# baurst/liso

Hardware: AMD Instinct MI355X
Metric: LISO train-step frames/sec (120k-pt clouds) (higher is better)
Workload: dtype bf16 (detector, BASELINE configs[2]) + f32 via bf16x3 MFMA (SLIM); north_star's 1e-3 on logits / flow is met by `parity_leg` (f32 via bf16x3 MFMA everywhere) and `fp32_exact_leg`, not by the bf16 detector

## Files before the change

liso_amd/csrc/conv_mfma.hip:

```cpp
#include <hip/hip_runtime.h>
#include <stdint.h>
#include <stdlib.h>

#include "../../include/liso_conv.h"
#include "../../include/liso_iou3d.h"
#include "conv_plan.h"
#include "dev_common.h"
#include "elem16.h"
#include "pack_chunk.h"
#include "per_device.h"

namespace {

using liso_dev::check_launch;

typedef __bf16 bf8 __attribute__((ext_vector_type(8)));
typedef float f16v __attribute__((ext_vector_type(16)));

__device__ __forceinline__ int xcd_remap(int bid, int total) {
    const int q = total >> 3, r = total & 7;
    const int xcd = bid & 7, idx = bid >> 3;
    return (xcd < r ? xcd * (q + 1) : r * (q + 1) + (xcd - r) * q) + idx;
}

using liso_pack::pack_bf16;
using liso_pack::round_bf16;
__device__ __forceinline__ float bf16_lo(unsigned w) { return __uint_as_float(w << 16); }
__device__ __forceinline__ float bf16_hi(unsigned w) { return __uint_as_float(w & 0xffff0000u); }

__device__ __forceinline__ bf8 as_bf8(const uint4& v) { return __builtin_bit_cast(bf8, v); }

template <typename E, int MI, int NJ, bool OUT_F32, bool WAVE_STATS = false>
__device__ __forceinline__ void conv_epilogue(const liso_conv_desc& d, const FwdArgs& a, f16v (&acc)[MI][NJ], int cls, int b, int tx, int ty,
                                              int wave, int r, int h, bool active, int n0, int stats_row, int tid_all,
                                              unsigned char* smem) {
    constexpr int BNT = 32 * NJ;
    constexpr int TH = 4 * MI;
    const int tid = tid_all & (kThreads - 1);
    const int grp = active ? 0 : 1;
    const bool want_stats = a.stats != nullptr;
    float s1[NJ], s2[NJ];
    const int ooy = d.class_ooy[cls], oox = d.class_oox[cls];
    const int col_stride = d.osx * d.y_pix_stride;
    unsigned colmask = 0;
#pragma unroll
    for (int e = 0; e < 16; e++) {
        const int vx = tx * 32 + (e & 3) + 8 * (e >> 2) + 4 * h;
        if (vx < d.wv && vx * d.osx + oox < d.wo) colmask |= 1u << e;
    }
    const int col0 = (tx * 32 + 4 * h) * d.osx + oox;
#pragma unroll
    for (int j = 0; j < NJ; j++) {
        s1[j] = 0.0f;
        s2[j] = 0.0f;
    }
#pragma unroll
    for (int i = 0; i < MI; i++) {
        const int vy = ty * TH + wave * MI + i;
        const int oy = vy * d.osy + ooy;
        const unsigned rowmask = (grp == 0 && vy < d.hv && oy < d.ho) ? colmask : 0u;
        if constexpr (WAVE_STATS) {
#pragma unroll
            for (int j = 0; j < NJ; j++) {
                s1[j] = 0.0f;
                s2[j] = 0.0f;
            }
        }
        const long row_base = (((long)b * d.ho + oy) * d.wo + col0) * d.y_pix_stride + d.y_ch_off;
#pragma unroll
        for (int j = 0; j < NJ; j++) {
            const int n = n0 + j * 32 + r;
            const bool n_ok = n < d.co;
            const float bias_v = (a.bias && n_ok) ? a.bias[n] : 0.0f;
            const float shift_v = (a.stats_shift && n_ok) ? a.stats_shift[n] : 0.0f;
            float v[16];
#pragma unroll
            for (int e = 0; e < 16; e++) {
                float val = acc[i][j][e] + bias_v;
                if (d.out_relu) val = fmaxf(val, 0.0f);
                if constexpr (!OUT_F32) val = E::round(val);
                v[e] = val;
                if constexpr (!WAVE_STATS) {
                    if (want_stats && ((rowmask >> e) & 1u)) {
                        const float dd = val - shift_v;
                        s1[j] += dd;
                        s2[j] = fmaf(dd, dd, s2[j]);
                    }
                }
            }
            if constexpr (WAVE_STATS) {
                if (want_stats) {
                    float q1[16], q2[16];
#pragma unroll
                    for (int e = 0; e < 16; e++) {
                        const float dd = ((rowmask >> e) & 1u) ? v[e] - shift_v : 0.0f;
                        q1[e] = dd;
                        q2[e] = dd * dd;
                    }
#pragma unroll
                    for (int w = 8; w >= 1; w >>= 1)
#pragma unroll
                        for (int e = 0; e < w; e++) {
                            q1[e] += q1[e + w];
                            q2[e] += q2[e + w];
                        }
                    s1[j] = q1[0];
                    s2[j] = q2[0];
                }
            }
            if constexpr (OUT_F32) {
                float* yg = (float*)a.y + row_base + n;
#pragma unroll
                for (int e = 0; e < 16; e++)
                    if (((rowmask >> e) & 1u) && n_ok) yg[((e & 3) + 8 * (e >> 2)) * col_stride] = v[e];
            } else {
                unsigned short* yg = (unsigned short*)a.y + row_base;
                const bool odd = r & 1;
                const int n_even = n & ~1;
                if ((d.y_pix_stride | d.y_ch_off) & 1) {
#pragma unroll
                    for (int e = 0; e < 16; e++)
                        if (((rowmask >> e) & 1u) && n_ok)
                            yg[((e & 3) + 8 * (e >> 2)) * col_stride + n] = (unsigned short)(E::pack(v[e], 0.0f) & 0xffffu);
                } else {
#pragma unroll
                    for (int e = 0; e < 16; e += 2) {
                        const float send = odd ? v[e] : v[e + 1];
                        const float recv = __int_as_float(__builtin_amdgcn_mov_dpp(__float_as_int(send), 0xB1, 0xF, 0xF, true));
                        const float c_lo = odd ? recv : v[e];
                        const float c_hi = odd ? v[e + 1] : recv;
                        const int ee = odd ? e + 1 : e;
                        const int koff = odd ? ((e + 1) & 3) + 8 * ((e + 1) >> 2) : (e & 3) + 8 * (e >> 2);
                        if ((rowmask >> ee) & 1u) {
                            unsigned short* dst = yg + koff * col_stride + n_even;
                            if (n_even + 1 < d.co)
                                *reinterpret_cast<unsigned*>(dst) = E::pack(c_lo, c_hi);
                            else if (n_even < d.co)
                                *dst = (unsigned short)(E::pack(c_lo, 0.0f) & 0xffffu);
                        }
                    }
                }
            }
        }
        if constexpr (WAVE_STATS) {
            if (want_stats) {
                float* red = reinterpret_cast<float*>(smem);
#pragma unroll
                for (int j = 0; j < NJ; j++) {
                    const float t1 = s1[j] + __shfl_xor(s1[j], 32);
                    const float t2 = s2[j] + __shfl_xor(s2[j], 32);
                    if (h == 0) {
                        red[((wave * MI + i) * BNT + j * 32 + r) * 2 + 0] = t1;
                        red[((wave * MI + i) * BNT + j * 32 + r) * 2 + 1] = t2;
                    }
                }
            }
        }
    }
    if constexpr (WAVE_STATS) {
    } else if (want_stats) {
        float* red = reinterpret_cast<float*>(smem);
#pragma unroll
        for (int j = 0; j < NJ; j++) {
            const float t1 = s1[j] + __shfl_xor(s1[j], 32);
            const float t2 = s2[j] + __shfl_xor(s2[j], 32);
            if (h == 0 && grp == 0) {
                red[(wave * BNT + j * 32 + r) * 2 + 0] = t1;
                red[(wave * BNT + j * 32 + r) * 2 + 1] = t2;
            }
        }
        __syncthreads();
        if (tid_all < BNT && n0 + tid < a.co_pad) {
            float q1 = 0.0f, q2 = 0.0f;
#pragma unroll
            for (int w = 0; w < 4; w++) {
                q1 += red[(w * BNT + tid) * 2 + 0];
                q2 += red[(w * BNT + tid) * 2 + 1];
            }
            a.stats[((long)stats_row * 2 + 0) * a.co_pad + n0 + tid] = q1;
            a.stats[((long)stats_row * 2 + 1) * a.co_pad + n0 + tid] = q2;
        }
    }
}
// ... 766 lines not shown
                }
            }
        };
        auto mul = [&](const Frag& F) {
#pragma unroll
            for (int kk = 0; kk < KS; kk++)
#pragma unroll
                for (int i = 0; i < MI; i++)
#pragma unroll
                    for (int j = 0; j < NJ; j++) {
                        if constexpr (X3) {
                            acc[i][j] = __builtin_amdgcn_mfma_f32_32x32x16_bf16(as_bf8(F.al[kk][i]), as_bf8(F.bh[kk][j]), acc[i][j], 0, 0, 0);
                            acc[i][j] = __builtin_amdgcn_mfma_f32_32x32x16_bf16(as_bf8(F.ah[kk][i]), as_bf8(F.bl[kk][j]), acc[i][j], 0, 0, 0);
                        }
                        acc[i][j] = E::mfma(F.ah[kk][i], F.bh[kk][j], acc[i][j]);
                    }
        };
#ifdef LISO_ROLES_STAMPS
        unsigned long long st_mul = 0, st_bar = 0, st_epi = 0, st_t;
        const unsigned long long st_k0 = __builtin_amdgcn_s_memtime();
#endif
        barrier();
#ifdef LISO_ROLES_STAMPS
        const unsigned long long st_k1 = __builtin_amdgcn_s_memtime();
#endif
        int k = 0;
        for (int j = 0; j < my_tiles; j++) {
#pragma unroll
            for (int i = 0; i < MI; i++)
#pragma unroll
                for (int jj = 0; jj < NJ; jj++)
#pragma unroll
                    for (int e = 0; e < 16; e++) acc[i][jj][e] = 0.0f;
            __builtin_amdgcn_s_setprio(2);
            for (int sl = 0; sl < nslab; sl++, k++) {
                const unsigned char* buf = base + (k & 1) * BUF;
                Frag F0, F1;
                STAMP_BEGIN
                read(buf, 0, F0);
#pragma unroll
                for (int tp = 0; tp < NTAPS; tp += 2) {
                    if (tp + 1 < NTAPS) read(buf, tp + 1, F1);
                    __builtin_amdgcn_sched_barrier(0);
                    mul(F0);
                    __builtin_amdgcn_sched_barrier(0);
                    if (tp + 1 < NTAPS) {
                        if (tp + 2 < NTAPS) read(buf, tp + 2, F0);
                        __builtin_amdgcn_sched_barrier(0);
                        mul(F1);
                        __builtin_amdgcn_sched_barrier(0);
                    }
                }
                STAMP_END(st_mul)
                barrier();
                STAMP_END(st_bar)
#ifndef LISO_ROLES_STAMPS
                if (sl == 0 && j > 0 && a.stats) {
                    const Tile P = tile_of(j - 1);
                    roles_flush_stats<MI, NJ>(a, P.b, P.ty, P.tx, P.n0, tid_all, smem);
                }
#endif
            }
            __builtin_amdgcn_s_setprio(0);
            const Tile T = tile_of(j);
#ifdef LISO_ROLES_STAMPS
            FwdArgs a2 = a;
            a2.stats = nullptr;
            conv_epilogue<E, MI, NJ, OUT_F32, true>(d, a2, acc, 0, T.b, T.tx, T.ty, wave, r, h, true, T.n0, T.row, tid_all, smem);
            STAMP_END(st_epi)
#else
            if (a.wide_out)
                roles_epilogue<E, MI, NJ, OUT_F32>(d, a, acc, T.b, T.tx, T.ty, wave, lane, T.n0, smem, base + 2 * BUF + wave * 2048);
            else
                conv_epilogue<E, MI, NJ, OUT_F32, true>(d, a, acc, 0, T.b, T.tx, T.ty, wave, r, h, true, T.n0, T.row, tid_all, smem);
#endif
        }
#ifndef LISO_ROLES_STAMPS
        if (a.stats) {
            barrier();
            const Tile P = tile_of(my_tiles - 1);
            roles_flush_stats<MI, NJ>(a, P.b, P.ty, P.tx, P.n0, tid_all, smem);
        }
#else
        if (a.stats) barrier();
#endif
#ifdef LISO_ROLES_STAMPS
        if (a.stats && tid_all == 0) {
            unsigned long long* o = reinterpret_cast<unsigned long long*>(a.stats) + (size_t)blockIdx.x * 16;
            o[0] = st_k1 - st_k0; o[1] = st_mul; o[2] = st_bar; o[3] = __builtin_amdgcn_s_memtime() - st_k0; o[4] = st_epi;
        }
#endif
    }
}

template <int MODE, int MI, int NJ, bool OUT_F32, bool PRO>
__global__ __launch_bounds__(kThreads, 2) void conv_1x1_kernel(const liso_conv_desc d, const FwdArgs a) {
    using E = typename liso_e16::Elem<MODE>::T;
    constexpr bool X3 = MODE == LISO_CONV_F32X3;
    constexpr int BNT = 32 * NJ;
    constexpr int TH = 4 * MI;
    constexpr int ES = X3 ? 4 : 2;
    __shared__ __attribute__((aligned(16))) unsigned char smem[4 * 96 * 2 * 4];
    __shared__ int s_dy[LISO_CONV_MAX_TAPS], s_dx[LISO_CONV_MAX_TAPS], s_w[LISO_CONV_MAX_TAPS];
    const int tid_all = threadIdx.x, wave = tid_all >> 6, lane = tid_all & 63, r = lane & 31, h = lane >> 5;
    if (tid_all < d.n_taps) {
        s_dy[tid_all] = d.tap_dy[tid_all];
        s_dx[tid_all] = d.tap_dx[tid_all];
        s_w[tid_all] = d.tap_w[tid_all];
    }
    int t = xcd_remap(blockIdx.x, a.total);
    const int nt = t % a.n_nt;
    t /= a.n_nt;
    const int tx = t % a.tiles_x;
    t /= a.tiles_x;
    const int ty = t % a.tiles_y;
    t /= a.tiles_y;
    const int b = t % d.batch;
    const int cls = t / d.batch;
    const int stats_row = ((cls * d.batch + b) * a.tiles_y + ty) * a.tiles_x + tx;
    const int n0 = nt * BNT;
    const int tap0 = d.n_classes > 1 ? cls : 0, tap1 = d.n_classes > 1 ? cls + 1 : d.n_taps;
    const unsigned char* xb = (const unsigned char*)a.x + (long)b * d.hi * d.wi * d.x_pix_stride * ES;
    int by[MI];
    bool okv[MI];
    const int bx = (tx * 32 + r) * d.isx;
#pragma unroll
    for (int i = 0; i < MI; i++) {
        const int vy = ty * TH + wave * MI + i;
        okv[i] = vy < d.hv && tx * 32 + r < d.wv;
        by[i] = vy * d.isy;
    }
    const unsigned short* wg = (const unsigned short*)a.w;
    const int kgroups = a.ci_pad >> 3;
    const long plane_elems = (long)d.w_taps * kgroups * a.co_pad * 8;
    int wn[NJ];
    bool okn[NJ];
#pragma unroll
    for (int j = 0; j < NJ; j++) {
        const int n = n0 + j * 32 + r;
        okn[j] = n < a.co_pad;
        wn[j] = (okn[j] ? n : 0) * 8;
    }
    const int aff = b * d.in_affine_batch_stride;
    __syncthreads();
    struct Frag {
        uint4 x[MI][X3 ? 2 : 1];
        float4 sc[2], sh[2];
        uint4 bh[NJ], bl[X3 ? NJ : 1];
        unsigned ok;
    };
    const int K = a.ci_pad;
    const int n_steps = (tap1 - tap0) * (K >> 4);
    int cur_tap = tap0, cur_k = 0;
    auto load = [&](Frag& F) {
        const int c = cur_k + 8 * h;
        const bool v0 = c < d.ci, v1 = c + 4 < d.ci;
        const int c_lo = v0 ? c : 0, c_hi = v1 ? c + 4 : 0;
        const int dy = s_dy[cur_tap], dx = s_dx[cur_tap];
        const int ix = bx + dx;
        unsigned ok = (v0 ? 256u : 0u) | (v1 ? 512u : 0u);
#pragma unroll
        for (int i = 0; i < MI; i++) {
            const int iy = by[i] + dy;
            const bool in = okv[i] && (unsigned)iy < (unsigned)d.hi && (unsigned)ix < (unsigned)d.wi;
            ok |= in ? (1u << i) : 0u;
            const unsigned char* px = xb + (in ? ((long)iy * d.wi + ix) * d.x_pix_stride : 0) * ES;
            F.x[i][0] = *reinterpret_cast<const uint4*>(px + c_lo * ES);
            if constexpr (X3) F.x[i][1] = *reinterpret_cast<const uint4*>(px + c_hi * ES);
        }
        F.ok = ok;
        if constexpr (PRO) {
            F.sc[0] = *reinterpret_cast<const float4*>(a.in_scale + aff + c_lo);
            F.sc[1] = *reinterpret_cast<const float4*>(a.in_scale + aff + c_hi);
            F.sh[0] = *reinterpret_cast<const float4*>(a.in_shift + aff + c_lo);
            F.sh[1] = *reinterpret_cast<const float4*>(a.in_shift + aff + c_hi);
        }
        const long ko = ((long)s_w[cur_tap] * kgroups + (cur_k >> 3) + h) * a.co_pad * 8;
#pragma unroll
        for (int j = 0; j < NJ; j++) {
            F.bh[j] = *reinterpret_cast<const uint4*>(wg + ko + wn[j]);
            if constexpr (X3) F.bl[j] = *reinterpret_cast<const uint4*>(wg + plane_elems + ko + wn[j]);
        }
        if (cur_k + 16 < K) {
            cur_k += 16;
        } else if (cur_tap + 1 < tap1) {
            cur_tap++;
            cur_k = 0;
        }
    };
    f16v acc[MI][NJ];
#pragma unroll
    for (int i = 0; i < MI; i++)
#pragma unroll
        for (int j = 0; j < NJ; j++)
#pragma unroll
            for (int e = 0; e < 16; e++) acc[i][j][e] = 0.0f;
    auto mul = [&](const Frag& F) {
        const bool v0 = (F.ok >> 8) & 1u, v1 = (F.ok >> 9) & 1u;
        uint4 ah[MI], al[X3 ? MI : 1];
#pragma unroll
        for (int i = 0; i < MI; i++) {
            const bool in = (F.ok >> i) & 1u;
            float f[8];
            if constexpr (X3) {
                const uint4 q0 = F.x[i][0], q1 = F.x[i][1];
                const unsigned w[8] = {q0.x, q0.y, q0.z, q0.w, q1.x, q1.y, q1.z, q1.w};
#pragma unroll
                for (int e = 0; e < 8; e++) f[e] = __uint_as_float(w[e]);
            } else {
                const uint4 q0 = F.x[i][0];
                const unsigned w[4] = {q0.x, q0.y, q0.z, q0.w};
#pragma unroll
                for (int e = 0; e < 4; e++) {
                    f[2 * e] = E::lo(w[e]);
                    f[2 * e + 1] = E::hi(w[e]);
                }
            }
            if constexpr (PRO) {
                const float sc[8] = {F.sc[0].x, F.sc[0].y, F.sc[0].z, F.sc[0].w, F.sc[1].x, F.sc[1].y, F.sc[1].z, F.sc[1].w};
                const float sh[8] = {F.sh[0].x, F.sh[0].y, F.sh[0].z, F.sh[0].w, F.sh[1].x, F.sh[1].y, F.sh[1].z, F.sh[1].w};
#pragma unroll
                for (int e = 0; e < 8; e++) {
                    f[e] = fmaf(f[e], sc[e], sh[e]);
                    if (d.in_relu) f[e] = fmaxf(f[e], 0.0f);
                }
            }
#pragma unroll
            for (int e = 0; e < 8; e++)
                if (!(in && (e < 4 ? v0 : v1))) f[e] = 0.0f;
            unsigned hi[4];
#pragma unroll
            for (int e = 0; e < 4; e++) hi[e] = E::pack(f[2 * e], f[2 * e + 1]);
            ah[i] = make_uint4(hi[0], hi[1], hi[2], hi[3]);
            if constexpr (X3) {
                unsigned lo[4];
#pragma unroll
                for (int e = 0; e < 4; e++) lo[e] = pack_bf16(f[2 * e] - bf16_lo(hi[e]), f[2 * e + 1] - bf16_hi(hi[e]));
                al[i] = make_uint4(lo[0], lo[1], lo[2], lo[3]);
            }
        }
#pragma unroll
        for (int j = 0; j < NJ; j++) {
            const uint4 bh = okn[j] ? F.bh[j] : make_uint4(0u, 0u, 0u, 0u);
            uint4 bl = make_uint4(0u, 0u, 0u, 0u);
            if constexpr (X3) bl = okn[j] ? F.bl[j] : make_uint4(0u, 0u, 0u, 0u);
#pragma unroll
            for (int i = 0; i < MI; i++) {
                if constexpr (X3) {
                    acc[i][j] = __builtin_amdgcn_mfma_f32_32x32x16_bf16(as_bf8(al[i]), as_bf8(bh), acc[i][j], 0, 0, 0);
                    acc[i][j] = __builtin_amdgcn_mfma_f32_32x32x16_bf16(as_bf8(ah[i]), as_bf8(bl), acc[i][j], 0, 0, 0);
                }
                acc[i][j] = E::mfma(ah[i], bh, acc[i][j]);
            }
        }
    };
    Frag F0, F1;
    load(F0);
    for (int s_ = 0; s_ < n_steps; s_ += 2) {
        load(F1);
        __builtin_amdgcn_sched_barrier(0);
        mul(F0);
        __builtin_amdgcn_sched_barrier(0);
        if (s_ + 1 < n_steps) {
            load(F0);
            __builtin_amdgcn_sched_barrier(0);
            mul(F1);
            __builtin_amdgcn_sched_barrier(0);
        }
    }
    conv_epilogue<E, MI, NJ, OUT_F32>(d, a, acc, cls, b, tx, ty, wave, r, h, true, n0, stats_row, tid_all, smem);
}

template <int NJ, bool PRO>
__global__ __launch_bounds__(kThreads, 2) void conv_taps_kernel(const liso_conv_desc d, const FwdArgs a) {
    constexpr int BNT = 32 * NJ;
    __shared__ __attribute__((aligned(16))) unsigned char smem[4 * 96 * 2 * 4];
    __shared__ int s_dy[LISO_CONV_MAX_TAPS + 1], s_dx[LISO_CONV_MAX_TAPS + 1], s_w[LISO_CONV_MAX_TAPS + 1];
    const int tid_all = threadIdx.x, wave = tid_all >> 6, lane = tid_all & 63, r = lane & 31, h = lane >> 5;
    if (tid_all <= d.n_taps && tid_all <= LISO_CONV_MAX_TAPS) {
        const bool real = tid_all < d.n_taps;
        s_dy[tid_all] = real ? d.tap_dy[tid_all] : (1 << 28);
        s_dx[tid_all] = real ? d.tap_dx[tid_all] : (1 << 28);
        s_w[tid_all] = real ? d.tap_w[tid_all] : 0;
    }
    int t = xcd_remap(blockIdx.x, a.total);
    const int nt = t % a.n_nt;
    t /= a.n_nt;
    const int tx = t % a.tiles_x;
    t /= a.tiles_x;
    const int ty = t % a.tiles_y;
    const int b = t / a.tiles_y;
    const int stats_row = (b * a.tiles_y + ty) * a.tiles_x + tx;
    const int n0 = nt * BNT;
    const int vy = ty * 4 + wave, vx = tx * 32 + r;
    const bool okv = vy < d.hv && vx < d.wv;
    const int by = vy * d.isy, bx = vx * d.isx;
    const float* xb = (const float*)a.x + (long)b * d.hi * d.wi * d.x_pix_stride;
    const unsigned short* wg = (const unsigned short*)a.w;
    const int kgroups = a.ci_pad >> 3;
    const long plane_elems = (long)d.w_taps * kgroups * a.co_pad * 8;
    int wn[NJ];
    bool okn[NJ];
#pragma unroll
    for (int j = 0; j < NJ; j++) {
        const int n = n0 + j * 32 + r;
        okn[j] = n < a.co_pad;
        wn[j] = (okn[j] ? n : 0) * 8;
    }
    const bool c1 = d.ci > 4;
    float sc[8], sh[8];
    if constexpr (PRO) {
        const int aff = b * d.in_affine_batch_stride;
#pragma unroll
        for (int e = 0; e < 8; e++) {
            const bool ok = e < d.ci;
            sc[e] = ok ? a.in_scale[aff + e] : 0.0f;
            sh[e] = ok ? a.in_shift[aff + e] : 0.0f;
        }
    }
    __syncthreads();
    struct Frag {
        float4 x[2];
        uint4 bh[NJ], bl[NJ];
        bool ok;
    };
    const int NS = (d.n_taps + 1) >> 1;
    auto load = [&](int s_, Frag& F) {
        const int tap = 2 * s_ + h;
        const int iy = by + s_dy[tap], ix = bx + s_dx[tap];
        F.ok = okv && (unsigned)iy < (unsigned)d.hi && (unsigned)ix < (unsigned)d.wi;
        const float* px = xb + (F.ok ? ((long)iy * d.wi + ix) * d.x_pix_stride : 0);
        F.x[0] = *reinterpret_cast<const float4*>(px);
        F.x[1] = *reinterpret_cast<const float4*>(px + (c1 ? 4 : 0));
        const long ko = (long)s_w[tap] * kgroups * a.co_pad * 8;
#pragma unroll
        for (int j = 0; j < NJ; j++) {
            F.bh[j] = *reinterpret_cast<const uint4*>(wg + ko + wn[j]);
            F.bl[j] = *reinterpret_cast<const uint4*>(wg + plane_elems + ko + wn[j]);
        }
    };
    f16v acc[1][NJ];
#pragma unroll
    for (int j = 0; j < NJ; j++)
#pragma unroll
        for (int e = 0; e < 16; e++) acc[0][j][e] = 0.0f;
    auto mul = [&](int s_, const Frag& F) {
        const bool real = 2 * s_ + h < d.n_taps;
        float f[8] = {F.x[0].x, F.x[0].y, F.x[0].z, F.x[0].w, F.x[1].x, F.x[1].y, F.x[1].z, F.x[1].w};
        if constexpr (PRO) {
#pragma unroll
            for (int e = 0; e < 8; e++) {
                f[e] = fmaf(f[e], sc[e], sh[e]);
                if (d.in_relu) f[e] = fmaxf(f[e], 0.0f);
            }
        }
#pragma unroll
        for (int e = 0; e < 8; e++)
            if (!(F.ok && real && (e < 4 || c1))) f[e] = 0.0f;
        unsigned hi[4], lo[4];
#pragma unroll
        for (int e = 0; e < 4; e++) {
            hi[e] = pack_bf16(f[2 * e], f[2 * e + 1]);
            lo[e] = pack_bf16(f[2 * e] - bf16_lo(hi[e]), f[2 * e + 1] - bf16_hi(hi[e]));
        }
        const uint4 ah = make_uint4(hi[0], hi[1], hi[2], hi[3]), al = make_uint4(lo[0], lo[1], lo[2], lo[3]);
#pragma unroll
        for (int j = 0; j < NJ; j++) {
            const bool okb = okn[j] && real;
            const uint4 bh = okb ? F.bh[j] : make_uint4(0u, 0u, 0u, 0u), bl = okb ? F.bl[j] : make_uint4(0u, 0u, 0u, 0u);
            acc[0][j] = __builtin_amdgcn_mfma_f32_32x32x16_bf16(as_bf8(al), as_bf8(bh), acc[0][j], 0, 0, 0);
            acc[0][j] = __builtin_amdgcn_mfma_f32_32x32x16_bf16(as_bf8(ah), as_bf8(bl), acc[0][j], 0, 0, 0);
            acc[0][j] = __builtin_amdgcn_mfma_f32_32x32x16_bf16(as_bf8(ah), as_bf8(bh), acc[0][j], 0, 0, 0);
        }
    };
    Frag F0, F1, F2;
    auto at = [&](int s_) { return s_ < NS ? s_ : NS - 1; };
    load(0, F0);
    load(at(1), F1);
    for (int s_ = 0; s_ < NS; s_ += 3) {
        load(at(s_ + 2), F2);
        __builtin_amdgcn_sched_barrier(0);
        mul(s_, F0);
        __builtin_amdgcn_sched_barrier(0);
        if (s_ + 1 < NS) {
            load(at(s_ + 3), F0);
            __builtin_amdgcn_sched_barrier(0);
            mul(s_ + 1, F1);
            __builtin_amdgcn_sched_barrier(0);
        }
        if (s_ + 2 < NS) {
            load(at(s_ + 4), F1);
            __builtin_amdgcn_sched_barrier(0);
            mul(s_ + 2, F2);
            __builtin_amdgcn_sched_barrier(0);
        }
    }
    conv_epilogue<liso_e16::Bf16, 1, NJ, true>(d, a, acc, 0, b, tx, ty, wave, r, h, true, n0, stats_row, tid_all, smem);
}

using liso_pack::kPackBf16;
using liso_pack::kPackF16;
using liso_pack::kPackF32;
using liso_pack::pack_chunks;
using liso_pack::pack_format;

__device__ __forceinline__ void pack_chunk(const float* __restrict__ src, int d1, int taps, int swap_ab, int K, int N, int Kp, int Np,
                                           int fmt, unsigned short* __restrict__ dst, long q) {
    const int n = (int)(q % Np);
    long t = q / Np;
    const int kcs = Kp / liso_pack::pack_chunk_k(fmt);
    const int kc = (int)(t % kcs);
    t /= kcs;
    const int tap = (int)(t % taps);
    const int plane = (int)(t / taps);
    liso_pack::pack_chunk_at(
        [&](int k, int nn, int tp) {
            if (k >= K || nn >= N) return 0.0f;
            const int ia = swap_ab ? k : nn, ib = swap_ab ? nn : k;
            return src[((long)ia * d1 + ib) * taps + tp];
        },
        fmt, plane, tap, kc, n, taps, Kp, Np, dst);
}
// ... 511 lines not shown
```

liso_amd/csrc/conv_plan.h:

```cpp
#ifndef LISO_CONV_PLAN_H
#define LISO_CONV_PLAN_H
#include <stdint.h>
#include <stdlib.h>

#include "../../include/liso_conv.h"

namespace {

constexpr int kThreads = 256;

struct FwdArgs {
    const void* x;
    const void* w;
    const float* bias;
    const float* in_scale;
    const float* in_shift;
    void* y;
    float* stats;
    const float* stats_shift;
    int ci_pad, co_pad;
    int cs;
    int g_taps;
    int cls_dy0[LISO_CONV_MAX_CLASSES], cls_dx0[LISO_CONV_MAX_CLASSES];
    int cls_inh[LISO_CONV_MAX_CLASSES], cls_inw[LISO_CONV_MAX_CLASSES];
    int tiles_x, tiles_y, n_nt, total;
    int x_plane_bytes;
    int pipelined;
    int slab_pipelined;
    int group_bytes;
    const float* occ;
    int roles;
    int wide_out;
    unsigned long long roles_tapw;
    int direct1x1;
    int direct_taps;
};

int round_up(int v, int m) { return (v + m - 1) / m * m; }

struct Plan {
    int mi, nj, cs, g, lds, sk;
    FwdArgs a;
};

int g_shared_gpu = 0;
int g_roles_cus = 0;

void plan_roles(const liso_conv_desc& d, Plan* p) {
    FwdArgs& a = p->a;
    a.roles = 0;
    static const int roles_env = getenv("LISO_CONV_ROLES") ? atoi(getenv("LISO_CONV_ROLES")) : 1;
    if (!roles_env || d.mode == LISO_CONV_F32) return;
    if (d.n_classes != 1 || d.isy != 1 || d.isx != 1 || d.osy != 1 || d.osx != 1 || d.n_taps != 9) return;
    const bool x3 = d.mode == LISO_CONV_F32X3;
    if (!x3 && d.ci % 32) return;
    int y0 = 1 << 30, x0 = 1 << 30, y1 = -(1 << 30), x1 = -(1 << 30);
    for (int t = 0; t < 9; t++) {
        y0 = d.tap_dy[t] < y0 ? d.tap_dy[t] : y0;
        y1 = d.tap_dy[t] > y1 ? d.tap_dy[t] : y1;
        x0 = d.tap_dx[t] < x0 ? d.tap_dx[t] : x0;
        x1 = d.tap_dx[t] > x1 ? d.tap_dx[t] : x1;
    }
    if (y1 - y0 != 2 || x1 - x0 != 2) return;
    int seen = 0;
    a.roles_tapw = 0ull;
    for (int t = 0; t < 9; t++) {
        const int pos = (d.tap_dy[t] - y0) * 3 + (d.tap_dx[t] - x0);
        if (d.tap_w[t] < 0 || d.tap_w[t] > 15) return;
        seen |= 1 << pos;
        a.roles_tapw |= (unsigned long long)d.tap_w[t] << (4 * pos);
    }
    if (seen != 0x1ff) return;
    const int cs = x3 ? 16 : 32, ks = cs / 16, nslab = (d.ci + cs - 1) / cs;
    if (nslab < 2) return;
    static const int force_mi = getenv("LISO_ROLES_MI") ? atoi(getenv("LISO_ROLES_MI")) : 0;
    static const int force_nj = getenv("LISO_ROLES_NJ") ? atoi(getenv("LISO_ROLES_NJ")) : 0;
    double best = 1e300;
    int bmi = 0, bnj = 0;
    for (int mi = 1; mi <= 2; mi++)
        for (int nj = 1; nj <= (x3 ? 3 : 2); nj++) {
            if (mi == 2 && nj == 3) continue;
            if ((force_mi && mi != force_mi) || (force_nj && nj != force_nj)) continue;
            const long blocks = (long)d.batch * ((d.hv + 4 * mi - 1) / (4 * mi)) * ((d.wv + 31) / 32) * ((d.co + 32 * nj - 1) / (32 * nj));
            const long rounds = (blocks + 255) / 256;
            const int npix = (4 * mi + 2) * 34, xb = (npix * 4 + 255) / 256, wb = (9 * (x3 ? 2 : 1) * (cs / 8) * 32 * nj + 255) / 256;
            const double mfma = 9.0 * ks * mi * nj * (x3 ? 3 : 1) * 32.0;
            const double load = 40.0 * (xb * (x3 ? 6 : 2) + wb * 2) + 200.0;
            const double cost = (double)rounds * (nslab * (mfma > load ? mfma : load) + 3000.0) - 1e-3 * mi * nj;
            if (cost < best) {
                best = cost;
                bmi = mi;
                bnj = nj;
            }
        }
    if (!bmi) return;
    a.roles = 1;
    p->mi = bmi;
    p->nj = bnj;
    p->sk = 1;
    p->cs = cs;
    a.cs = cs;
    a.cls_dy0[0] = y0;
    a.cls_dx0[0] = x0;
    const int bnt = 32 * bnj, th = 4 * bmi;
    a.n_nt = (d.co + bnt - 1) / bnt;
    a.tiles_x = (d.wv + 31) / 32;
    a.tiles_y = (d.hv + th - 1) / th;
    a.total = d.batch * a.tiles_y * a.tiles_x * a.n_nt;
    const int planes = x3 ? 2 : 1;
    const int buf = ((th + 2) * 34 * (cs * 2 + 16) * planes + 9 * planes * (cs / 8) * bnt * 16 + 15) / 16 * 16;
    p->lds = 4096 + 2 * buf + 4 * 2048;
    const bool of32 = x3 || d.out_f32;
    const int cv = of32 ? 4 : 8;
    a.wide_out = (d.co % cv == 0 && d.y_pix_stride % cv == 0 && d.y_ch_off % cv == 0) ? 1 : 0;
}

inline int direct_panel_width(int co) {
    int best = 1, best_cost = 1 << 30;
    for (int nj = 1; nj <= 3; nj++) {
        const int cost = ((co + 32 * nj - 1) / (32 * nj)) * (2 + nj);
        if (cost < best_cost) {
            best_cost = cost;
            best = nj;
        }
    }
    return best;
}

void plan_1x1(const liso_conv_desc& d, Plan* p) {
    FwdArgs& a = p->a;
    a.direct1x1 = 0;
    if (d.mode != LISO_CONV_F32X3 && d.mode != LISO_CONV_BF16) return;
    if (d.n_classes > 1) {
        if (d.n_taps != d.n_classes) return;
        for (int c = 0; c < d.n_classes; c++)
            if (d.class_tap_begin[c] != c) return;
    } else if (d.osy != 1 || d.osx != 1) {
        return;
    }
    bool cell = d.n_classes == 1 && d.n_taps > 1 && d.n_taps == d.isy * d.isx;
    if (cell) {
        unsigned seen = 0;
        for (int t = 0; t < d.n_taps && cell; t++) {
            if (d.tap_dy[t] < 0 || d.tap_dy[t] >= d.isy || d.tap_dx[t] < 0 || d.tap_dx[t] >= d.isx) cell = false;
            else seen |= 1u << (d.tap_dy[t] * d.isx + d.tap_dx[t]);
        }
        cell = cell && d.n_taps <= 16 && seen == (1u << d.n_taps) - 1u;
    }
    const bool strided = d.n_classes == 1 && d.n_taps == 9 && d.isy == 2 && d.isx == 2 && d.ci > 8 &&
                         d.ci * (d.mode == LISO_CONV_F32X3 ? 4 : 2) <= 256;
    if (d.n_classes == 1 && d.n_taps != 1 && !cell && !strided) return;
    if (a.roles) return;
    for (int t = 0; t < d.n_taps; t++)
        if (d.tap_w[t] < 0 || d.tap_w[t] >= d.w_taps) return;
    if (d.in_affine_batch_stride & 3) return;
    a.roles = 0;
    const int nj = direct_panel_width(d.co);
    const long tiles4 = (long)d.n_classes * d.batch * ((d.hv + 3) / 4) * ((d.wv + 31) / 32) * ((d.co + 32 * nj - 1) / (32 * nj));
    const int mi = tiles4 >= 1024 ? 2 : 1;
    a.direct1x1 = 1;
    p->mi = mi;
    p->nj = nj;
    p->sk = 1;
    const int bnt = 32 * nj, th = 4 * mi;
    a.n_nt = (d.co + bnt - 1) / bnt;
    a.tiles_x = (d.wv + 31) / 32;
    a.tiles_y = (d.hv + th - 1) / th;
    a.total = d.n_classes * d.batch * a.tiles_y * a.tiles_x * a.n_nt;
}

void plan_taps(const liso_conv_desc& d, Plan* p) {
    FwdArgs& a = p->a;
    a.direct_taps = 0;
    if (a.roles || a.direct1x1 || d.mode != LISO_CONV_F32X3 || d.n_classes != 1 || d.n_taps < 2 || d.ci > 8 || d.osy != 1 || d.osx != 1)
        return;
    if (d.in_affine_batch_stride & 3) return;
    for (int t = 0; t < d.n_taps; t++)
        if (d.tap_w[t] < 0 || d.tap_w[t] >= d.w_taps) return;
    const int nj = direct_panel_width(d.co);
    a.direct_taps = 1;
    p->mi = 1;
    p->nj = nj;
    p->sk = 1;
    const int bnt = 32 * nj;
    a.n_nt = (d.co + bnt - 1) / bnt;
    a.tiles_x = (d.wv + 31) / 32;
    a.tiles_y = (d.hv + 3) / 4;
    a.total = d.batch * a.tiles_y * a.tiles_x * a.n_nt;
}

bool make_plan(const liso_conv_desc& d, Plan* p) {
    if (d.mode == LISO_CONV_F16) {
        liso_conv_desc e = d;
        e.mode = LISO_CONV_BF16;
        return make_plan(e, p);
    }
    if (d.batch <= 0 || d.ci <= 0 || d.co <= 0 || d.n_classes < 1 || d.n_classes > LISO_CONV_MAX_CLASSES) return false;
    if (d.n_taps < 1 || d.n_taps > LISO_CONV_MAX_TAPS || d.class_tap_begin[0] != 0 || d.class_tap_begin[d.n_classes] != d.n_taps)
        return false;
    if (d.mode != LISO_CONV_BF16 && d.mode != LISO_CONV_F32X3 && d.mode != LISO_CONV_F32) return false;
    const bool x3 = d.mode == LISO_CONV_F32X3, f32 = d.mode == LISO_CONV_F32, fin = x3 || f32;
    const int vec = fin ? 4 : 8;
    if (d.ci % vec || d.x_pix_stride % vec || d.x_pix_stride < d.ci) return false;
    const int planes = x3 ? 2 : 1;
    auto pix_bytes = [&](int cs) { return (f32 ? cs * 4 : cs * 2) + 16; };
    auto panel_bytes = [&](int cs, int bnt) { return f32 ? (cs / 4) * bnt * 16 : planes * (cs / 8) * bnt * 16; };
    FwdArgs& a = p->a;
    a.ci_pad = round_up(d.ci, 16);
    a.co_pad = round_up(d.co, 64);
    p->nj = d.co <= 32 ? 1 : 2;
    {
        const long tiles4 = (long)d.n_classes * d.batch * ((d.hv + 3) / 4) * ((d.wv + 31) / 32);
        if (p->nj == 2 && tiles4 * ((d.co + 63) / 64) < 160) p->nj = 1;
    }
    const int bnt = 32 * p->nj;
    a.n_nt = (d.co + bnt - 1) / bnt;
    auto blocks = [&](int th) { return (long)d.n_classes * d.batch * ((d.hv + th - 1) / th) * ((d.wv + 31) / 32) * a.n_nt; };
    int max_taps = 1;
    for (int c = 0; c < d.n_classes; c++) {
        const int nt = d.class_tap_begin[c + 1] - d.class_tap_begin[c];
        if (nt < 1) return false;
        max_taps = nt > max_taps ? nt : max_taps;
        for (int t = d.class_tap_begin[c]; t < d.class_tap_begin[c + 1]; t++)
            if (d.tap_w[t] < 0 || d.tap_w[t] >= d.w_taps) return false;
    }
    auto tile_pixels = [&](int th, int* inh, int* inw, int* y0s, int* x0s) {
        int max_pix = 0;
        for (int c = 0; c < d.n_classes; c++) {
            int y0 = 1 << 30, y1 = -(1 << 30), x0 = 1 << 30, x1 = -(1 << 30);
            for (int t = d.class_tap_begin[c]; t < d.class_tap_begin[c + 1]; t++) {
                y0 = d.tap_dy[t] < y0 ? d.tap_dy[t] : y0;
                y1 = d.tap_dy[t] > y1 ? d.tap_dy[t] : y1;
                x0 = d.tap_dx[t] < x0 ? d.tap_dx[t] : x0;
                x1 = d.tap_dx[t] > x1 ? d.tap_dx[t] : x1;
            }
            y0s[c] = y0;
            x0s[c] = x0;
            inh[c] = (th - 1) * d.isy + (y1 - y0) + 1;
            inw[c] = 31 * d.isx + (x1 - x0) + 1;
            const int np = inh[c] * inw[c];
            max_pix = np > max_pix ? np : max_pix;
        }
        return max_pix;
    };
    int mi_first = blocks(8) >= 512 ? 2 : 1;
    if (const char* e = getenv("LISO_CONV_MI")) mi_first = atoi(e) == 2 ? 2 : atoi(e) == 1 ? 1 : mi_first;
    const int cs_opts[2] = {fin ? 32 : 64, fin ? 16 : 32};
    long best = -1;
    const bool few_blocks = !g_shared_gpu && blocks(4 * mi_first) <= 256;
    for (int pass = 0; pass < 2 && best < 0; pass++) {
        const int cap = (pass == 0 && !few_blocks ? 79 : 158) * 1024;
        for (int mi = mi_first; mi >= 1; mi--) {
            int inh[LISO_CONV_MAX_CLASSES], inw[LISO_CONV_MAX_CLASSES], y0s[LISO_CONV_MAX_CLASSES], x0s[LISO_CONV_MAX_CLASSES];
            const int max_pix = tile_pixels(4 * mi, inh, inw, y0s, x0s);
            for (int k = 0; k < 2; k++) {
                const int cs = cs_opts[k];
                if (k == 0 && cs_opts[1] >= a.ci_pad) continue;
                const int xb = round_up(max_pix * pix_bytes(cs), 16);
                const int panel = panel_bytes(cs, bnt);
                int g = (cap - 512 - xb * planes) / panel;
                if (g < 1) continue;
                g = g > max_taps ? max_taps : g;
                const long score = ((long)g * (cs / 16) * mi * 1000) + cs + (mi == mi_first ? 500000 : 0);
                if (score > best) {
                    best = score;
                    p->mi = mi;
                    p->cs = cs;
                    p->g = g;
                    a.x_plane_bytes = xb;
                    p->lds = 512 + xb * planes + g * panel;
                    for (int c = 0; c < d.n_classes; c++) {
                        a.cls_dy0[c] = y0s[c];
                        a.cls_dx0[c] = x0s[c];
                        a.cls_inh[c] = inh[c];
                        a.cls_inw[c] = inw[c];
                    }
                }
            }
            if (best >= 0) break;
        }
    }
    if (best < 0) return false;
    if (p->lds < 4096) p->lds = 4096;
    const int th = 4 * p->mi;
    a.cs = p->cs;
    a.g_taps = p->g;
    {
        int max_pix = 0;
        for (int c = 0; c < d.n_classes; c++) max_pix = a.cls_inh[c] * a.cls_inw[c] > max_pix ? a.cls_inh[c] * a.cls_inw[c] : max_pix;
        const int cpp = fin ? p->cs / 4 : p->cs / 8;
        const int x_chunks = (max_pix * cpp + kThreads - 1) / kThreads;
        const int w_chunks = (max_taps * (panel_bytes(p->cs, bnt) / 16) + kThreads - 1) / kThreads;
        const int panel = panel_bytes(p->cs, bnt);
        int g_pipe = (10 * kThreads * 16) / panel;
        g_pipe = g_pipe > p->g ? p->g : g_pipe;
        a.slab_pipelined = (p->g >= max_taps && x_chunks <= 12 && w_chunks <= 10) ? 1 : 0;
        a.pipelined = (x_chunks <= 12 && g_pipe >= 1) ? 1 : 0;
        if (a.pipelined && !(a.slab_pipelined && p->g >= max_taps)) {
            p->g = g_pipe;
            a.g_taps = g_pipe;
            p->lds = 512 + a.x_plane_bytes * planes + g_pipe * panel;
            if (p->lds < 4096) p->lds = 4096;
        }
    }
    a.tiles_x = (d.wv + 31) / 32;
    a.tiles_y = (d.hv + th - 1) / th;
    a.total = (int)blocks(th);
    p->sk = 1;
    a.group_bytes = round_up(a.x_plane_bytes * planes + max_taps * panel_bytes(p->cs, bnt), 16);
    if (x3 && a.slab_pipelined && p->mi == 1 && p->nj == 1 && a.total <= 256 && d.ci > p->cs && 512 + 2 * a.group_bytes <= 160 * 1024 &&
        a.group_bytes >= 16 * kThreads * 4)
        p->sk = 2;
// ... 11 lines not shown
```

Baseline: 1038.

## Hoist per-tap address math, streamline bf16 packing, restructure direct-conv load/mul pipeline

```diff
diff --git a/liso_amd/csrc/conv_mfma.hip b/liso_amd/csrc/conv_mfma.hip
--- a/liso_amd/csrc/conv_mfma.hip
+++ b/liso_amd/csrc/conv_mfma.hip
@@ -29,6 +29,13 @@
 __device__ __forceinline__ float bf16_hi(unsigned w) { return __uint_as_float(w & 0xffff0000u); }
 
 __device__ __forceinline__ bf8 as_bf8(const uint4& v) { return __builtin_bit_cast(bf8, v); }
+
+typedef float f2v __attribute__((ext_vector_type(2)));
+typedef __bf16 bf2v __attribute__((ext_vector_type(2)));
+__device__ __forceinline__ unsigned pack2_bf16(float a, float b) {
+    const f2v v = {a, b};
+    return __builtin_bit_cast(unsigned, __builtin_convertvector(v, bf2v));
+}
 
 template <typename E, int MI, int NJ, bool OUT_F32, bool WAVE_STATS = false>
 __device__ __forceinline__ void conv_epilogue(const liso_conv_desc& d, const FwdArgs& a, f16v (&acc)[MI][NJ], int cls, int b, int tx, int ty,
@@ -1101,40 +1108,55 @@
     const int K = a.ci_pad;
     const int n_steps = (tap1 - tap0) * (K >> 4);
     int cur_tap = tap0, cur_k = 0;
+    long pix[MI];
+    unsigned tap_ok = 0;
+    long w_tap = 0;
+    int wl[NJ];
+#pragma unroll
+    for (int j = 0; j < NJ; j++) wl[j] = wn[j] + h * a.co_pad * 8;
+    auto enter_tap = [&]() {
+        const int dy = __builtin_amdgcn_readfirstlane(s_dy[cur_tap]), dx = __builtin_amdgcn_readfirstlane(s_dx[cur_tap]);
+        const int ix = bx + dx;
+        tap_ok = 0;
+#pragma unroll
+        for (int i = 0; i < MI; i++) {
+            const int iy = by[i] + dy;
+            const bool in = okv[i] && (unsigned)iy < (unsigned)d.hi && (unsigned)ix < (unsigned)d.wi;
+            tap_ok |= in ? (1u << i) : 0u;
+            pix[i] = (in ? ((long)iy * d.wi + ix) * d.x_pix_stride : 0) * ES;
+        }
+        w_tap = (long)__builtin_amdgcn_readfirstlane(s_w[cur_tap]) * kgroups * a.co_pad * 8;
+    };
+    enter_tap();
     auto load = [&](Frag& F) {
         const int c = cur_k + 8 * h;
         const bool v0 = c < d.ci, v1 = c + 4 < d.ci;
         const int c_lo = v0 ? c : 0, c_hi = v1 ? c + 4 : 0;
-        const int dy = s_dy[cur_tap], dx = s_dx[cur_tap];
-        const int ix = bx + dx;
-        unsigned ok = (v0 ? 256u : 0u) | (v1 ? 512u : 0u);
 #pragma unroll
         for (int i = 0; i < MI; i++) {
-            const int iy = by[i] + dy;
-            const bool in = okv[i] && (unsigned)iy < (unsigned)d.hi && (unsigned)ix < (unsigned)d.wi;
-            ok |= in ? (1u << i) : 0u;
-            const unsigned char* px = xb + (in ? ((long)iy * d.wi + ix) * d.x_pix_stride : 0) * ES;
+            const unsigned char* px = xb + pix[i];
             F.x[i][0] = *reinterpret_cast<const uint4*>(px + c_lo * ES);
             if constexpr (X3) F.x[i][1] = *reinterpret_cast<const uint4*>(px + c_hi * ES);
         }
-        F.ok = ok;
+        F.ok = tap_ok | (v0 ? 256u : 0u) | (v1 ? 512u : 0u);
         if constexpr (PRO) {
             F.sc[0] = *reinterpret_cast<const float4*>(a.in_scale + aff + c_lo);
             F.sc[1] = *reinterpret_cast<const float4*>(a.in_scale + aff + c_hi);
             F.sh[0] = *reinterpret_cast<const float4*>(a.in_shift + aff + c_lo);
             F.sh[1] = *reinterpret_cast<const float4*>(a.in_shift + aff + c_hi);
         }
-        const long ko = ((long)s_w[cur_tap] * kgroups + (cur_k >> 3) + h) * a.co_pad * 8;
+        const unsigned short* wk = wg + w_tap + (long)(cur_k >> 3) * a.co_pad * 8;
 #pragma unroll
         for (int j = 0; j < NJ; j++) {
-            F.bh[j] = *reinterpret_cast<const uint4*>(wg + ko + wn[j]);
-            if constexpr (X3) F.bl[j] = *reinterpret_cast<const uint4*>(wg + plane_elems + ko + wn[j]);
+            F.bh[j] = *reinterpret_cast<const uint4*>(wk + wl[j]);
+            if constexpr (X3) F.bl[j] = *reinterpret_cast<const uint4*>(wk + plane_elems + wl[j]);
         }
         if (cur_k + 16 < K) {
             cur_k += 16;
         } else if (cur_tap + 1 < tap1) {
             cur_tap++;
             cur_k = 0;
+            enter_tap();
         }
     };
     f16v acc[MI][NJ];
@@ -1150,73 +1172,90 @@
 #pragma unroll
         for (int i = 0; i < MI; i++) {
             const bool in = (F.ok >> i) & 1u;
-            float f[8];
-            if constexpr (X3) {
-                const uint4 q0 = F.x[i][0], q1 = F.x[i][1];
-                const unsigned w[8] = {q0.x, q0.y, q0.z, q0.w, q1.x, q1.y, q1.z, q1.w};
-#pragma unroll
-                for (int e = 0; e < 8; e++) f[e] = __uint_as_float(w[e]);
+            if constexpr (!X3 && !PRO) {
+                const uint4 q0 = F.x[i][0];
+                const bool m0 = in && v0, m1 = in && v1;
+                ah[i] = make_uint4(m0 ? q0.x : 0u, m0 ? q0.y : 0u, m1 ? q0.z : 0u, m1 ? q0.w : 0u);
             } else {
-                const uint4 q0 = F.x[i][0];
-                const unsigned w[4] = {q0.x, q0.y, q0.z, q0.w};
-#pragma unroll
-                for (int e = 0; e < 4; e++) {
-                    f[2 * e] = E::lo(w[e]);
-                    f[2 * e + 1] = E::hi(w[e]);
-                }
-            }
-            if constexpr (PRO) {
-                const float sc[8] = {F.sc[0].x, F.sc[0].y, F.sc[0].z, F.sc[0].w, F.sc[1].x, F.sc[1].y, F.sc[1].z, F.sc[1].w};
-                const float sh[8] = {F.sh[0].x, F.sh[0].y, F.sh[0].z, F.sh[0].w, F.sh[1].x, F.sh[1].y, F.sh[1].z, F.sh[1].w};
-#pragma unroll
-                for (int e = 0; e < 8; e++) {
-                    f[e] = fmaf(f[e], sc[e], sh[e]);
-                    if (d.in_relu) f[e] = fmaxf(f[e], 0.0f);
-                }
-            }
-#pragma unroll
-            for (int e = 0; e < 8; e++)
-                if (!(in && (e < 4 ? v0 : v1))) f[e] = 0.0f;
-            unsigned hi[4];
-#pragma unroll
-            for (int e = 0; e < 4; e++) hi[e] = E::pack(f[2 * e], f[2 * e + 1]);
-            ah[i] = make_uint4(hi[0], hi[1], hi[2], hi[3]);
-            if constexpr (X3) {
-                unsigned lo[4];
-#pragma unroll
-                for (int e = 0; e < 4; e++) lo[e] = pack_bf16(f[2 * e] - bf16_lo(hi[e]), f[2 * e + 1] - bf16_hi(hi[e]));
-                al[i] = make_uint4(lo[0], lo[1], lo[2], lo[3]);
+                float f[8];
+                if constexpr (X3) {
+                    const uint4 q0 = F.x[i][0], q1 = F.x[i][1];
+                    const unsigned w[8] = {q0.x, q0.y, q0.z, q0.w, q1.x, q1.y, q1.z, q1.w};
+#pragma unroll
+                    for (int e = 0; e < 8; e++) f[e] = __uint_as_float(w[e]);
+                } else {
+                    const uint4 q0 = F.x[i][0];
+                    const unsigned w[4] = {q0.x, q0.y, q0.z, q0.w};
+#pragma unroll
+                    for (int e = 0; e < 4; e++) {
+                        f[2 * e] = E::lo(w[e]);
+                        f[2 * e + 1] = E::hi(w[e]);
+                    }
+                }
+                if constexpr (PRO) {
+                    const float sc[8] = {F.sc[0].x, F.sc[0].y, F.sc[0].z, F.sc[0].w, F.sc[1].x, F.sc[1].y, F.sc[1].z, F.sc[1].w};
+                    const float sh[8] = {F.sh[0].x, F.sh[0].y, F.sh[0].z, F.sh[0].w, F.sh[1].x, F.sh[1].y, F.sh[1].z, F.sh[1].w};
+#pragma unroll
+                    for (int e = 0; e < 8; e++) {
+                        f[e] = fmaf(f[e], sc[e], sh[e]);
+                        if (d.in_relu) f[e] = fmaxf(f[e], 0.0f);
+                    }
+                }
+                auto pack = [](float lo_v, float hi_v) {
+                    if constexpr (MODE == LISO_CONV_F16) return E::pack(lo_v, hi_v);
+                    else return pack2_bf16(lo_v, hi_v);
+                };
+                unsigned hi[4];
+                if constexpr (X3) {
+#pragma unroll
+                    for (int e = 0; e < 8; e++)
+                        if (!(in && (e < 4 ? v0 : v1))) f[e] = 0.0f;
+#pragma unroll
+                    for (int e = 0; e < 4; e++) hi[e] = pack(f[2 * e], f[2 * e + 1]);
+                    unsigned lo[4];
+#pragma unroll
+                    for (int e = 0; e < 4; e++) lo[e] = pack(f[2 * e] - bf16_lo(hi[e]), f[2 * e + 1] - bf16_hi(hi[e]));
+                    al[i] = make_uint4(lo[0], lo[1], lo[2], lo[3]);
+                } else {
+#pragma unroll
+                    for (int e = 0; e < 4; e++) hi[e] = (in && (e < 2 ? v0 : v1)) ? pack(f[2 * e], f[2 * e + 1]) : 0u;
+                }
+                ah[i] = make_uint4(hi[0], hi[1], hi[2], hi[3]);
             }
         }
 #pragma unroll
         for (int j = 0; j < NJ; j++) {
-            const uint4 bh = okn[j] ? F.bh[j] : make_uint4(0u, 0u, 0u, 0u);
-            uint4 bl = make_uint4(0u, 0u, 0u, 0u);
-            if constexpr (X3) bl = okn[j] ? F.bl[j] : make_uint4(0u, 0u, 0u, 0u);
 #pragma unroll
             for (int i = 0; i < MI; i++) {
                 if constexpr (X3) {
-                    acc[i][j] = __builtin_amdgcn_mfma_f32_32x32x16_bf16(as_bf8(al[i]), as_bf8(bh), acc[i][j], 0, 0, 0);
-                    acc[i][j] = __builtin_amdgcn_mfma_f32_32x32x16_bf16(as_bf8(ah[i]), as_bf8(bl), acc[i][j], 0, 0, 0);
-                }
-                acc[i][j] = E::mfma(ah[i], bh, acc[i][j]);
+                    acc[i][j] = __builtin_amdgcn_mfma_f32_32x32x16_bf16(as_bf8(al[i]), as_bf8(F.bh[j]), acc[i][j], 0, 0, 0);
+                    acc[i][j] = __builtin_amdgcn_mfma_f32_32x32x16_bf16(as_bf8(ah[i]), as_bf8(F.bl[j]), acc[i][j], 0, 0, 0);
+                }
+                acc[i][j] = E::mfma(ah[i], F.bh[j], acc[i][j]);
             }
         }
     };
-    Frag F0, F1;
-    load(F0);
-    for (int s_ = 0; s_ < n_steps; s_ += 2) {
-        load(F1);
+    constexpr int D = 2;
+    Frag F[D];
+#pragma unroll
+    for (int q = 0; q < D; q++) load(F[q]);
+    int s_ = 0;
+    for (; s_ + D < n_steps; s_ += D) {
+#pragma unroll
+        for (int q = 0; q < D; q++) {
+            __builtin_amdgcn_sched_barrier(0);
+            mul(F[q]);
+            __builtin_amdgcn_sched_barrier(0);
+            load(F[q]);
+        }
+    }
+    const int rem = n_steps - s_;
+#pragma unroll
+    for (int q = 0; q < D; q++) {
         __builtin_amdgcn_sched_barrier(0);
-        mul(F0);
-        __builtin_amdgcn_sched_barrier(0);
-        if (s_ + 1 < n_steps) {
-            load(F0);
-            __builtin_amdgcn_sched_barrier(0);
-            mul(F1);
-            __builtin_amdgcn_sched_barrier(0);
-        }
-    }
+        if (q < rem) mul(F[q]);
+    }
+    __builtin_amdgcn_sched_barrier(0);
     conv_epilogue<E, MI, NJ, OUT_F32>(d, a, acc, cls, b, tx, ty, wave, r, h, true, n0, stats_row, tid_all, smem);
 }
 
diff --git a/liso_amd/csrc/conv_plan.h b/liso_amd/csrc/conv_plan.h
--- a/liso_amd/csrc/conv_plan.h
+++ b/liso_amd/csrc/conv_plan.h
@@ -115,6 +115,8 @@
     a.wide_out = (d.co % cv == 0 && d.y_pix_stride % cv == 0 && d.y_ch_off % cv == 0) ? 1 : 0;
 }
 
+constexpr int kDirectCus = 256;
+
 inline int direct_panel_width(int co) {
     int best = 1, best_cost = 1 << 30;
     for (int nj = 1; nj <= 3; nj++) {
@@ -155,9 +157,11 @@
         if (d.tap_w[t] < 0 || d.tap_w[t] >= d.w_taps) return;
     if (d.in_affine_batch_stride & 3) return;
     a.roles = 0;
-    const int nj = direct_panel_width(d.co);
-    const long tiles4 = (long)d.n_classes * d.batch * ((d.hv + 3) / 4) * ((d.wv + 31) / 32) * ((d.co + 32 * nj - 1) / (32 * nj));
+    int nj = direct_panel_width(d.co);
+    const long pix_tiles4 = (long)d.n_classes * d.batch * ((d.hv + 3) / 4) * ((d.wv + 31) / 32);
+    const long tiles4 = pix_tiles4 * ((d.co + 32 * nj - 1) / (32 * nj));
     const int mi = tiles4 >= 1024 ? 2 : 1;
+    if (nj == 3 && pix_tiles4 * ((d.co + 95) / 96) < kDirectCus) nj = 2;
     a.direct1x1 = 1;
     p->mi = mi;
     p->nj = nj;
```

Result: no change. 1042 (median of 6 runs) (+0.4%).
